# b-g-goodell/lattice-cryptography

Measured on NVIDIA B200. Metric: LM-OTS verifies/sec, higher is better.
Workload: dtype u32 (mod-q integer arithmetic, q < 2^16)

## Files before the change

lattice_cryptography_b200/csrc/api.cu:

```cuda
#include <cstdio>
#include <cstring>
#include <new>
#include <algorithm>
#include <cstdlib>
#include <string>
#include <vector>

#include <nvtx3/nvToolsExt.h>

#include "../../include/lcb200.h"
#include "engine.h"

using namespace lcb;

struct lcb_ctx {
    int device = 0;
    cudaStream_t stream = nullptr;
    bool own_stream = false;
    cudaStream_t copy_stream = nullptr;
    int secpar = 0, q = 0, d = 0, l = 0, rou = 0;
    RingCtx ring{};
    bool generic = false;
    bool wide = false;
    GenCtx gen{};
    uint32_t* d_gen_tab = nullptr;
    NttTables* d_tab = nullptr;
    uint32_t* d_a_hat = nullptr;
    bool has_key_ch = false;
    std::string last_error;
    int64_t launches = 0;
    uint8_t* idx_scratch = nullptr;
    size_t idx_scratch_bytes = 0;
    uint2* il_scratch = nullptr;
    size_t il_scratch_bytes = 0;
    uint32_t* d_mod_tab = nullptr;
    uint32_t* coop_scratch = nullptr;
    size_t coop_scratch_bytes = 0;
    bool profile = false;
    struct Pending { int id; cudaEvent_t a, b; };
    std::vector<Pending> pending;
    double prof_ms[24] = {0};
    int64_t prof_n[24] = {0};
};

namespace {

struct NvtxRange {
    explicit NvtxRange(const char* name) { nvtxRangePushA(name); }
    ~NvtxRange() { nvtxRangePop(); }
};
#define LCB_RANGE() NvtxRange nvtx_range_(__func__)

thread_local std::string g_create_error;

int fail(lcb_ctx* c, int status, const std::string& what) {
    if (c) c->last_error = what;
    return status;
}

int fail_cuda(lcb_ctx* c, cudaError_t e, const char* what) {
    return fail(c, e == cudaErrorMemoryAllocation ? LCB_ERR_OOM : LCB_ERR_CUDA,
                std::string(what) + ": " + cudaGetErrorString(e));
}

#define CK(c, call)                                              \
    do {                                                         \
        cudaError_t e_ = (call);                                 \
        if (e_ != cudaSuccess) return fail_cuda((c), e_, #call); \
    } while (0)

constexpr int64_t kPipeChunk = 1 << 17;

enum KernelId { K_SAMPLER = 0, K_SHAKE, K_NTT_FWD, K_NTT_INV, K_POLY_MUL, K_MATVEC, K_SIGN, K_VERIFY, K_ADDSUB,
                K_AGG_COEFS, K_AGG_PARTIAL, K_AGG_FINISH, K_AGGV_PARTIAL, K_AGGV_FINISH, K_PACK, K_UNPACK, K_GROUP_IDS,
                K_AGG_COEFS_SEG, K_AGG_PARTIAL_SEG, K_AGGV_PARTIAL_SEG, K_AGGV_RESIDUES, K_AGGV_LIMITS, K_AGG_FINISH_PACK,
                K_COUNT };
const char* const kKernelNames[K_COUNT] = {"sampler", "shake256", "ntt_fwd", "ntt_inv", "poly_mul", "matvec", "sign",
                                           "verify", "vec_addsub", "agg_coefs", "agg_partial", "agg_finish",
                                           "aggv_partial", "aggv_finish", "pack", "unpack", "group_ids",
                                           "agg_coefs_seg", "agg_partial_seg", "aggv_partial_seg", "aggv_residues",
                                           "aggv_limits", "agg_finish_pack"};
// ... 706 lines not shown
    m.q4 = 4 * uq;
    m.in_off = m.cq + 26 * uq + FP_BIAS;
    m.in_off_q4 = m.in_off + m.q4;
    m.bias_mod_q = FP_BIAS % uq;
    m.z1c = (int32_t)t.w[1] > (int32_t)m.half ? (int32_t)t.w[1] - (int32_t)uq : (int32_t)t.w[1];
    m.k1 = (uint32_t)((((1ull << 30) + (1ull << 15) + uq - 1) / uq) * uq);
    {
        uint64_t inv = uq;
        for (int it = 0; it < 6; ++it) inv *= 2 - (uint64_t)uq * inv;
        m.qinv_lo = (uint32_t)inv;
        m.qinv_hi = (uint32_t)(inv >> 32);
        const uint64_t lim = ~0ull / uq;
        m.dlim_lo = (uint32_t)lim;
        m.dlim_hi = (uint32_t)(lim >> 32);
        m.kq18 = (((1u << 18) + uq - 1) / uq) * uq;
        m.kw0 = (uint32_t)((uint64_t)(0x4B400000u + 2u) * uq);
    }
    for (int k = 0; k < 16; ++k) {
        c->ring.sc.w[k] = t.w[k];
        c->ring.sc.ws[k] = t.ws[k];
        c->ring.sc.iw[k] = t.iw[k];
        c->ring.sc.iws[k] = t.iws[k];
        c->ring.scf.w[k] = t.w[k];
        c->ring.scf.wq[k] = t.f_wq[k];
        c->ring.scf.cst[k] = t.f_cst[k];
        c->ring.scf.kw[k] = t.f_kw[k];
    }
    if ((e = cudaMalloc(&c->d_tab, sizeof(NttTables))) != cudaSuccess) return bail(e, "cudaMalloc tables");
    if ((e = cudaMemcpy(c->d_tab, &t, sizeof(NttTables), cudaMemcpyHostToDevice)) != cudaSuccess) return bail(e, "cudaMemcpy tables");
    if ((e = cudaMalloc(&c->d_a_hat, (size_t)l * D * sizeof(uint32_t))) != cudaSuccess) return bail(e, "cudaMalloc key_ch");
    c->ring.tab = c->d_tab;
    c->ring.a_hat = c->d_a_hat;
    c->gen.a_hat = c->d_a_hat;
    c->ring.l = l;
    c->ring.num_sms = prop.multiProcessorCount;
    {
        std::vector<uint32_t> mt(SAMPLER_MOD_TABLE_WORDS);
        fill_sampler_mod_table(mt.data());
        if ((e = cudaMalloc(&c->d_mod_tab, mt.size() * sizeof(uint32_t))) != cudaSuccess) return bail(e, "cudaMalloc sampler tables");
        if ((e = cudaMemcpy(c->d_mod_tab, mt.data(), mt.size() * sizeof(uint32_t), cudaMemcpyHostToDevice)) != cudaSuccess)
            return bail(e, "cudaMemcpy sampler tables");
    }
    *out = c;
    return LCB_OK;
}

int lcb_ctx_destroy(lcb_ctx* c) {
    if (!c) return LCB_OK;
    cudaSetDevice(c->device);
    if (c->stream) cudaStreamSynchronize(c->stream);
    if (c->d_tab) cudaFree(c->d_tab);
    if (c->d_gen_tab) cudaFree(c->d_gen_tab);
    if (c->d_a_hat) cudaFree(c->d_a_hat);
    if (c->idx_scratch) cudaFree(c->idx_scratch);
    if (c->d_mod_tab) cudaFree(c->d_mod_tab);
    if (c->il_scratch) cudaFree(c->il_scratch);
    if (c->coop_scratch) cudaFree(c->coop_scratch);
    if (c->own_stream && c->stream) cudaStreamDestroy(c->stream);
    if (c->copy_stream) {
        cudaStreamSynchronize(c->copy_stream);
        cudaStreamDestroy(c->copy_stream);
    }
    delete c;
    return LCB_OK;
}

int lcb_ctx_set_stream(lcb_ctx* c, void* cuda_stream) {
    if (!c) return LCB_ERR_INVALID;
    CK(c, cudaSetDevice(c->device));
    CK(c, cudaStreamSynchronize(c->stream));
    if (c->own_stream) cudaStreamDestroy(c->stream);
    c->stream = static_cast<cudaStream_t>(cuda_stream);
    c->own_stream = false;
    return LCB_OK;
}

int lcb_synchronize(lcb_ctx* c) {
    if (!c) return LCB_ERR_INVALID;
    CK(c, cudaSetDevice(c->device));
    CK(c, cudaStreamSynchronize(c->stream));
    return LCB_OK;
}

int lcb_ctx_root_of_unity(const lcb_ctx* c) { return c ? c->rou : LCB_ERR_INVALID; }

int64_t lcb_launch_count(const lcb_ctx* c) { return c ? c->launches : 0; }

static int profile_drain(lcb_ctx* c) {
    if (c->pending.empty()) return LCB_OK;
    CK(c, cudaStreamSynchronize(c->stream));
    for (auto& p : c->pending) {
        float ms = 0.f;
        if (cudaEventElapsedTime(&ms, p.a, p.b) == cudaSuccess) {
            c->prof_ms[p.id] += ms;
            c->prof_n[p.id] += 1;
        }
        cudaEventDestroy(p.a);
        cudaEventDestroy(p.b);
    }
    c->pending.clear();
    return LCB_OK;
}

int lcb_profile_enable(lcb_ctx* c, int on) {
    if (!c) return LCB_ERR_INVALID;
    CK(c, cudaSetDevice(c->device));
    int st = profile_drain(c);
    c->profile = on != 0;
    return st;
}

int lcb_profile_reset(lcb_ctx* c) {
    if (!c) return LCB_ERR_INVALID;
    CK(c, cudaSetDevice(c->device));
    int st = profile_drain(c);
    for (int i = 0; i < K_COUNT; ++i) { c->prof_ms[i] = 0; c->prof_n[i] = 0; }
    return st;
}

int lcb_profile_read(lcb_ctx* c, const char* kernel, double* total_ms, int64_t* launches) {
    if (!c || !kernel || !total_ms || !launches) return LCB_ERR_INVALID;
    CK(c, cudaSetDevice(c->device));
    int st = profile_drain(c);
    if (st != LCB_OK) return st;
    for (int i = 0; i < K_COUNT; ++i)
        if (std::strcmp(kernel, kKernelNames[i]) == 0) {
            *total_ms = c->prof_ms[i];
            *launches = c->prof_n[i];
            return LCB_OK;
        }
    return fail(c, LCB_ERR_INVALID, std::string("unknown kernel name ") + kernel);
}

int lcb_set_key_ch(lcb_ctx* c, const int16_t* key_ch_coef) {
    LCB_RANGE();
    if (!c || !key_ch_coef) return LCB_ERR_INVALID;
    CK(c, cudaSetDevice(c->device));
    Staging sg(c);
    const size_t cnt = (size_t)c->l * c->d;
    const int16_t* d_in;
    CK(c, sg.in(&d_in, key_ch_coef, cnt * ew(c)));
    uint16_t* d_ntt;
    CK(c, sg.alloc((void**)&d_ntt, cnt * ew(c) * sizeof(uint16_t)));
    if (c->generic) CK(c, timed(c, K_NTT_FWD, [&] { return g_launch_ntt_fwd(c->gen, d_in, c->l, d_ntt, c->stream); }));
    else CK(c, timed(c, K_NTT_FWD, [&] { return launch_ntt_fwd(c->ring, d_in, c->l, d_ntt, c->stream); }));
    if (c->wide) {
        CK(c, cudaMemcpyAsync(c->d_a_hat, d_ntt, cnt * sizeof(uint32_t), cudaMemcpyDeviceToDevice, c->stream));
        CK(c, cudaStreamSynchronize(c->stream));
    } else {
        std::vector<uint16_t> h16(cnt);
        CK(c, cudaMemcpyAsync(h16.data(), d_ntt, h16.size() * sizeof(uint16_t), cudaMemcpyDeviceToHost, c->stream));
        CK(c, cudaStreamSynchronize(c->stream));
        std::vector<uint32_t> h32(h16.begin(), h16.end());
        CK(c, cudaMemcpyAsync(c->d_a_hat, h32.data(), h32.size() * sizeof(uint32_t), cudaMemcpyHostToDevice, c->stream));
        CK(c, cudaStreamSynchronize(c->stream));
    }
    c->has_key_ch = true;
    CK(c, sg.finish());
    return LCB_OK;
}

int lcb_shake256_batch(lcb_ctx* c, const uint8_t* in, const int64_t* in_off, int64_t n, uint8_t* out,
                       int64_t out_len) {
    LCB_RANGE();
    if (!c || !in_off || !out || n < 0 || out_len < 0) return LCB_ERR_INVALID;
    if (n == 0 || out_len == 0) return LCB_OK;
    CK(c, cudaSetDevice(c->device));
    int64_t total = 0;
    CK(c, last_offset(c, in, in_off, n, &total));
    Staging sg(c);
    const uint8_t* d_in;
    const int64_t* d_off;
    uint8_t* d_out;
    CK(c, sg.in(&d_in, in, (size_t)total));
    CK(c, sg.in(&d_off, in_off, (size_t)n + 1));
    CK(c, sg.out(&d_out, out, (size_t)(n * out_len)));
    CK(c, timed(c, K_SHAKE, [&] { return launch_shake256(d_in, d_off, n, d_out, out_len, c->stream); }));
    CK(c, sg.finish());
    return LCB_OK;
}

int lcb_expand_seeds(lcb_ctx* c, const uint8_t* secret32, int64_t first, int64_t n, uint8_t* seeds) {
    LCB_RANGE();
    if (!c || !secret32 || !seeds || n < 0 || first < 0) return LCB_ERR_INVALID;
    if (c->secpar > 512 || (c->secpar & 7)) return fail(c, LCB_ERR_INVALID, "seed expansion needs secpar to be a multiple of 8, at most 512");
    if (n == 0) return LCB_OK;
    CK(c, cudaSetDevice(c->device));
    Staging sg(c);
    uint8_t* d_secret;
    uint8_t* d_out;
    CK(c, sg.alloc((void**)&d_secret, 32, true));
    CK(c, cudaMemcpyAsync(d_secret, secret32, 32, cudaMemcpyDefault, c->stream));
    CK(c, sg.out(&d_out, seeds, (size_t)n * c->secpar, true));
    CK(c, timed(c, K_SHAKE, [&] { return launch_seed_expand(d_secret, first, n, c->secpar, d_out, c->stream); }));
    CK(c, sg.finish());
    if (!on_device(secret32)) CK(c, cudaStreamSynchronize(c->stream));
    return LCB_OK;
}

int lcb_hash2polyvec_batch(lcb_ctx* c, const char* salt, const uint8_t* msgs, const int64_t* msg_off, int64_t n,
                           int bd, int wt, int vec_len, int16_t* out_dense, int16_t* out_pairs) {
    LCB_RANGE();
    if (!c || !msg_off || n < 0) return LCB_ERR_INVALID;
    if (n == 0) return LCB_OK;
    CK(c, cudaSetDevice(c->device));
    SamplerArgs a{};
    int st = fill_sampler(c, a, salt, nullptr, bd, wt, vec_len);
    if (st != LCB_OK) return fail(c, st, "bad sampler parameters");
    int64_t total = 0;
    CK(c, last_offset(c, msgs, msg_off, n, &total));
// ... 179 lines not shown
    CK(c, sg.out(&d_sig, sig, (size_t)n * l * D_));
    CK(c, sg.alloc((void**)&d_pairs, (size_t)n * sch->ch_wt * 2 * ew(c) * sizeof(int16_t)));
    int st = run_challenge(c, sch, d_msg, d_off, n, d_pairs);
    if (st != LCB_OK) return st;
    CK(c, timed(c, K_SIGN, [&] {
        return c->generic ? g_launch_sign(c->gen, d_sk, d_pairs, sch->ch_wt, n, d_sig, c->stream)
                          : launch_sign(c->ring, d_sk, d_pairs, sch->ch_wt, n, d_sig, c->stream);
    }));
    CK(c, sg.finish());
    return LCB_OK;
}

int lcb_lm_verify_batch(lcb_ctx* c, const lcb_scheme* sch, const uint16_t* vk_ntt, const uint8_t* chmsg,
                        const int64_t* chmsg_off, const int16_t* sig, const uint16_t* st_ntt, int64_t n, int bd,
                        int wt, uint8_t* verdict) {
    LCB_RANGE();
    if (!c || !sch || !vk_ntt || !chmsg_off || !sig || !verdict || n < 0 || bd < 0 || wt < 0) return LCB_ERR_INVALID;
    if (!c->has_key_ch) return fail(c, LCB_ERR_NO_KEY_CH, "lcb_lm_verify_batch before lcb_set_key_ch");
    if (n > ((int64_t)1 << 30)) return fail(c, LCB_ERR_INVALID, "more than 2^30 items in one verify call");
    if (n == 0) return LCB_OK;
    CK(c, cudaSetDevice(c->device));
    const int l = c->l;
    int64_t total = 0;
    CK(c, last_offset(c, chmsg, chmsg_off, n, &total));
    Staging sg(c);
    const uint16_t *d_vk, *d_st;
    const uint8_t* d_msg;
    const int64_t* d_off;
    const int16_t* d_sig;
    int16_t* d_pairs;
    uint8_t* d_verdict;
    const size_t D_ = (size_t)c->d * ew(c);
    CK(c, sg.in(&d_vk, vk_ntt, (size_t)n * 2 * D_));
    CK(c, sg.in(&d_msg, chmsg, (size_t)total));
    CK(c, sg.in(&d_off, chmsg_off, (size_t)n + 1));
    bool piped = false;
    CK(c, sg.in_piped(&d_sig, sig, (size_t)n * l * D_, &piped));
    CK(c, sg.in(&d_st, st_ntt, (size_t)n * D_));
    CK(c, sg.out(&d_verdict, verdict, (size_t)n));
    CK(c, sg.alloc((void**)&d_pairs, (size_t)n * sch->ch_wt * 2 * ew(c) * sizeof(int16_t)));
    const int vbd = bd > 32767 ? 32767 : bd;
    const int64_t chunk = piped && n > kPipeChunk ? kPipeChunk : n;
    std::vector<cudaEvent_t> arrived;
    if (piped) {
        CK(c, sg.pipe_begin());
        for (int64_t first = 0; first < n; first += chunk) {
            const int64_t m = n - first < chunk ? n - first : chunk;
            cudaEvent_t ev;
            CK(c, sg.pipe_chunk(d_sig + (size_t)first * l * D_, sig + (size_t)first * l * D_,
                                (size_t)m * l * D_ * sizeof(int16_t), &ev));
            arrived.push_back(ev);
        }
    }
    for (int64_t first = 0, k = 0; first < n; first += chunk, ++k) {
        const int64_t m = n - first < chunk ? n - first : chunk;
        int16_t* pairs = d_pairs + (size_t)first * sch->ch_wt * 2 * ew(c);
        int st = run_challenge(c, sch, d_msg, d_off + first, m, pairs);
        if (st != LCB_OK) return st;
        if (piped) CK(c, cudaStreamWaitEvent(c->stream, arrived[k], 0));
        CK(c, timed(c, K_VERIFY, [&] {
            if (c->generic)
                return g_launch_verify(c->gen, d_sig + (size_t)first * l * D_, d_vk + (size_t)first * 2 * D_, pairs, sch->ch_wt,
                                       nullptr, d_st ? d_st + (size_t)first * D_ : nullptr, m, bd, wt, d_verdict + first, c->stream);
            return launch_verify(c->ring, d_sig + (size_t)first * l * D_, d_vk + (size_t)first * 2 * D_, pairs, sch->ch_wt,
                                 nullptr, d_st ? d_st + (size_t)first * D_ : nullptr, m, vbd, wt, d_verdict + first,
                                 c->stream);
        }));
    }
    CK(c, sg.finish());
    return LCB_OK;
}

int lcb_pack_batch(lcb_ctx* c, const void* values, int64_t npoly, int bits, int bias, uint8_t* packed,
                   uint8_t* in_range) {
    LCB_RANGE();
    if (!c || !values || !packed || npoly < 0 || bits < 1 || bits > 16 || bias < 0 || bias > 65535) return LCB_ERR_INVALID;
    if (c->generic) return fail(c, LCB_ERR_INVALID, "the packed wire format is defined for d == 256, q < 2^16 contexts only");
    if (npoly == 0) return LCB_OK;
    CK(c, cudaSetDevice(c->device));
    Staging sg(c);
    const uint16_t* d_in;
    uint8_t *d_out, *d_ok;
    CK(c, sg.in(&d_in, static_cast<const uint16_t*>(values), (size_t)npoly * D));
    CK(c, sg.out(&d_out, packed, (size_t)npoly * 32 * bits));
    CK(c, sg.out(&d_ok, in_range, (size_t)npoly));
    if (reinterpret_cast<uintptr_t>(d_out) & 3u) return fail(c, LCB_ERR_INVALID, "packed buffer must be 4-byte aligned");
    CK(c, timed(c, K_PACK, [&] { return launch_pack(c->ring, d_in, npoly, bits, bias, d_out, d_ok, c->stream); }));
    CK(c, sg.finish());
    return LCB_OK;
}

int lcb_unpack_batch(lcb_ctx* c, const uint8_t* packed, int64_t npoly, int bits, int bias, void* values) {
    LCB_RANGE();
    if (!c || !values || !packed || npoly < 0 || bits < 1 || bits > 16 || bias < 0 || bias > 65535) return LCB_ERR_INVALID;
    if (c->generic) return fail(c, LCB_ERR_INVALID, "the packed wire format is defined for d == 256, q < 2^16 contexts only");
    if (npoly == 0) return LCB_OK;
    CK(c, cudaSetDevice(c->device));
    Staging sg(c);
    const uint8_t* d_in;
    uint16_t* d_out;
    CK(c, sg.in(&d_in, packed, (size_t)npoly * 32 * bits));
    CK(c, sg.out(&d_out, static_cast<uint16_t*>(values), (size_t)npoly * D));
    if (reinterpret_cast<uintptr_t>(d_in) & 3u) return fail(c, LCB_ERR_INVALID, "packed buffer must be 4-byte aligned");
    CK(c, timed(c, K_UNPACK, [&] { return launch_unpack(c->ring, d_in, npoly, bits, bias, d_out, c->stream); }));
    CK(c, sg.finish());
    return LCB_OK;
}

}

namespace {

int verify_packed(lcb_ctx* c, const lcb_scheme* sch, const uint8_t* vk_packed, int vk_bits, const uint8_t* chmsg,
// ... 903 lines not shown
```

lattice_cryptography_b200/csrc/engine.h:

```cpp
#pragma once
#include <cstdint>
#include <cuda_runtime.h>
#include "lcb_device.cuh"

namespace lcb {

constexpr int SALT_BYTES = 48;

struct SamplerArgs {
    const uint8_t* msgs;
    const int64_t* off;
    int64_t n;
    int64_t shared_len;
    int64_t index_first;
    int shared_msg;
    alignas(8) uint8_t salt[SALT_BYTES];
    int salt_len;
    alignas(8) uint8_t salt2[SALT_BYTES];
    int salt2_len;
    int paired;
    int secpar, bd, wt, vec_len;
    int idx_bits;
    int mag_bits;
    int pad_bits;
// ... 50 lines not shown
    const uint32_t* a_hat;
    int l, num_sms;
    bool wide;
};

cudaError_t g_launch_ntt_fwd(const GenCtx& c, const void* coef, int64_t npoly, void* out, cudaStream_t st);
cudaError_t g_launch_ntt_inv(const GenCtx& c, const void* in, int64_t npoly, void* coef, cudaStream_t st);
cudaError_t g_launch_poly_mul(const GenCtx& c, const void* a, const void* b, int64_t npoly, void* out, cudaStream_t st);
cudaError_t g_launch_ref_repr(const GenCtx& c, const void* coef, int64_t npoly, void* out, cudaStream_t st);
cudaError_t g_launch_matvec(const GenCtx& c, const void* vec_coef, int64_t nvec, void* vec_ntt, void* y_ntt, void* y_coef,
                            cudaStream_t st);
cudaError_t g_launch_sign(const GenCtx& c, const void* sk_ntt, const void* ch_pairs, int ch_wt, int64_t n, void* sig,
                          cudaStream_t st);
cudaError_t g_launch_verify(const GenCtx& c, const void* vec_coef, const void* vk_ntt, const void* ch_pairs, int ch_wt,
                            const void* rhs_only, const void* extra_rhs, int64_t n, int64_t bd, int wt, uint8_t* verdict,
                            cudaStream_t st);
cudaError_t g_launch_vec_addsub(const GenCtx& c, const void* a, const void* b, int64_t nelem, int sub, void* out,
                                cudaStream_t st);
cudaError_t g_launch_agg_partial(const GenCtx& c, const void* sigs, const void* ag_pairs, int64_t count, void* partial,
                                 cudaStream_t st);
cudaError_t g_launch_agg_partial_poly(const GenCtx& c, const void* sigs, const void* ag_pairs, int ag_wt, int64_t count,
                                      void* partial, cudaStream_t st);
cudaError_t g_launch_aggv_partial_poly(const GenCtx& c, const void* vk_ntt, const void* ch_pairs, int ch_wt, const void* ag_pairs,
                                       int ag_wt, int64_t count, void* partial, cudaStream_t st);
cudaError_t g_launch_agg_finish(const GenCtx& c, const void* partial, void* ag_sig, cudaStream_t st);
cudaError_t g_launch_aggv_partial(const GenCtx& c, const void* vk_ntt, const void* ch_pairs, int ch_wt, const void* ag_pairs,
                                  int64_t count, void* partial, cudaStream_t st);
cudaError_t g_launch_aggv_finish(const GenCtx& c, const void* partial, const void* ag_sig, int64_t total, int64_t ag_cap,
                                 int64_t avf_bd, int avf_wt, uint8_t* verdict, cudaStream_t st);

struct RingCtx {
    ModQ m;
    StageConst sc;
    StageConstF scf;
    StageConstF iscf;
    const NttTables* tab;
    const uint32_t* a_hat;
    int l;
    int num_sms;
};

cudaError_t launch_ntt_fwd(const RingCtx& c, const int16_t* coef, int64_t npoly, uint16_t* out, cudaStream_t st);
cudaError_t launch_ntt_ref_repr(const RingCtx& c, const int16_t* coef, int64_t npoly, int16_t* out, cudaStream_t st);
cudaError_t launch_ntt_inv(const RingCtx& c, const uint16_t* in, int64_t npoly, int16_t* coef, cudaStream_t st);
cudaError_t launch_poly_mul(const RingCtx& c, const int16_t* a, const int16_t* b, int64_t npoly, int16_t* out,
                            cudaStream_t st);
cudaError_t launch_matvec(const RingCtx& c, const int16_t* vec_coef, int64_t nvec, uint16_t* vec_ntt,
                          uint16_t* y_ntt, int16_t* y_coef, cudaStream_t st);
cudaError_t launch_sign(const RingCtx& c, const uint16_t* sk_ntt, const int16_t* ch_pairs, int ch_wt, int64_t n,
                        int16_t* sig, cudaStream_t st);
cudaError_t launch_verify(const RingCtx& c, const int16_t* vec_coef, const uint16_t* vk_ntt,
                          const int16_t* ch_pairs, int ch_wt, const uint16_t* rhs_only, const uint16_t* extra_rhs,
                          int64_t n, int bd, int wt, uint8_t* verdict, cudaStream_t st);
cudaError_t launch_verify_packed(const RingCtx& c, const uint8_t* sig_packed, int sig_bits, int sig_bias,
                                 const uint8_t* vk_packed, int vk_bits, const int16_t* ch_pairs, int ch_wt, int64_t n,
                                 int bd, int wt, uint8_t* verdict, cudaStream_t st, const uint8_t* st_packed = nullptr);
cudaError_t launch_sign_packed(const RingCtx& c, const uint16_t* sk_ntt, const int16_t* ch_pairs, int ch_wt, int64_t n,
                               int sig_bits, int sig_bias, uint8_t* sig_packed, uint8_t* in_range, cudaStream_t st);
cudaError_t launch_vec_addsub(const RingCtx& c, const int16_t* a, const int16_t* b, int64_t nelem, int sub,
                              int16_t* out, cudaStream_t st);
cudaError_t launch_agg_partial(const RingCtx& c, const int16_t* sigs, const int16_t* ag_pairs, int64_t count,
                               int32_t* partial, cudaStream_t st);
cudaError_t launch_agg_finish(const RingCtx& c, const int32_t* partial, int16_t* ag_sig, cudaStream_t st);
cudaError_t launch_aggv_partial(const RingCtx& c, const uint16_t* vk_ntt, const int16_t* ch_pairs, int ch_wt,
                                const int16_t* ag_pairs, int64_t count, int32_t* partial, cudaStream_t st);
cudaError_t launch_aggv_finish(const RingCtx& c, const int32_t* partial, const int16_t* ag_sig, int64_t total,
                               int ag_cap, int avf_bd, int avf_wt, uint8_t* verdict, cudaStream_t st);
cudaError_t launch_agg_partial_seg(const RingCtx& c, const void* sigs, int sig_bits, int sig_bias, const int16_t* ag_pairs,
                                   const int32_t* gid, int64_t total, int64_t n_agg, int32_t* partial, cudaStream_t st);
cudaError_t launch_agg_finish_n(const RingCtx& c, const int32_t* partial, int64_t nelem, int16_t* ag_sig, cudaStream_t st);
cudaError_t launch_aggv_partial_seg(const RingCtx& c, const void* vk_ntt, int vk_bits, const int16_t* ch_pairs, int ch_wt,
                                    const int16_t* ag_pairs, const int32_t* gid, int64_t total, int64_t n_agg,
                                    int32_t* partial, cudaStream_t st);
cudaError_t launch_aggv_residues(const RingCtx& c, const int32_t* partial, int64_t nelem, uint16_t* out, cudaStream_t st);
cudaError_t launch_aggv_limits(const RingCtx& c, const int64_t* agg_off, int64_t n_agg, const int16_t* ag_sig, int64_t ag_cap,
                               uint8_t* verdict, cudaStream_t st);
cudaError_t launch_aggv_limits_packed(const RingCtx& c, const int64_t* agg_off, int64_t n_agg, const uint8_t* ag_packed, int bits,
                                      int bias, int64_t ag_cap, uint8_t* verdict, cudaStream_t st);
cudaError_t launch_verify_rhs_packed(const RingCtx& c, const uint8_t* vec_packed, int bits, int bias, const uint16_t* rhs_only,
                                     int64_t n, int bd, int wt, uint8_t* verdict, cudaStream_t st);

cudaError_t launch_pack(const RingCtx& c, const void* in, int64_t npoly, int bits, int bias, uint8_t* out,
                        uint8_t* in_range, cudaStream_t st);
cudaError_t launch_unpack(const RingCtx& c, const uint8_t* in, int64_t npoly, int bits, int bias, void* out,
                          cudaStream_t st);
cudaError_t launch_agg_finish_pack(const RingCtx& c, const int32_t* partial, int64_t npoly, int bits, int bias, uint8_t* out,
                                   uint8_t* in_range, cudaStream_t st);

}
```

lattice_cryptography_b200/csrc/ring.cu:

```cuda
#include <cstdlib>

#include "engine.h"

namespace lcb {

namespace {

constexpr int RBS = 128;
constexpr int HWB = RBS / LANES;
#ifdef LCB_EXP_MBS
constexpr int MBS = LCB_EXP_MBS;
#else
constexpr int MBS = 512;
#endif
constexpr int MHWB = MBS / LANES;

struct HalfWarp {
    int lane;
    int slot;
    uint32_t* xb;
    unsigned mask;
};

__device__ __forceinline__ HalfWarp half_warp(uint32_t* xbase) {
// ... 1099 lines not shown
                const uint32_t hi = w + 1 < words ? __ldg(p + w + 1) : 0u;
                nz = (__funnelshift_r(__ldg(p + w), hi, (unsigned)pos & 31u) & mask) != bias;
            }
            ok = nz;
        }
        if (!ok) verdict[g] = 0;
    }
}

__global__ void __launch_bounds__(32) k_aggv_finish(ModQ m, StageConst sc, const NttTables* __restrict__ tab,
                                                    const uint32_t* __restrict__ a_hat, int l,
                                                    const int32_t* __restrict__ partial,
                                                    const int16_t* __restrict__ ag_sig, int64_t total, int ag_cap,
                                                    int avf_bd, int avf_wt, uint8_t* __restrict__ verdict) {
    __shared__ __align__(16) uint32_t xbuf[XWARP];
    const HalfWarp h = half_warp(xbuf);
    LaneTw tw;
    load_lane_tw(tw, tab->w, tab->ws, h.lane);
    uint64_t acc[EPT];
#pragma unroll
    for (int i = 0; i < EPT; ++i) acc[i] = 0;
    int maxabs = 0, maxw = 0;
    for (int i = 0; i < l; ++i) {
        const int16_t* p = ag_sig + i * D;
        uint32_t r[EPT];
        int nz = 0;
#pragma unroll
        for (int j = 0; j < EPT; ++j) {
            int x = __ldg(p + h.lane + 16 * j);
            maxabs = max(maxabs, abs(x));
            nz += (x != 0);
            r[j] = (uint32_t)(x + (int)m.cq);
        }
#pragma unroll
        for (int o = 8; o >= 1; o >>= 1) nz += __shfl_xor_sync(0xFFFFFFFFu, nz, o);
        maxw = max(maxw, nz);
        ntt_fwd_256(r, m, sc, tw, h.xb, h.lane);
#pragma unroll
        for (int g = 0; g < EPT; ++g) acc[g] += (uint64_t)r[g] * __ldg(a_hat + i * D + 16 * h.lane + g);
    }
#pragma unroll
    for (int o = 8; o >= 1; o >>= 1) maxabs = max(maxabs, __shfl_xor_sync(0xFFFFFFFFu, maxabs, o));
    bool ok = maxabs >= 1 && maxabs <= avf_bd && maxw >= 1 && maxw <= avf_wt && total >= 1 && total <= ag_cap;
#pragma unroll
    for (int k = 0; k < EPT; ++k) {
        int v = partial[16 * h.lane + k] % (int)m.q;
        if (v < 0) v += (int)m.q;
        ok &= reduce64(acc[k], m) == (uint32_t)v;
    }
    const unsigned votes = __ballot_sync(0xFFFFFFFFu, ok);
    if (threadIdx.x == 0) verdict[0] = (votes & 0xFFFFu) == 0xFFFFu ? 1 : 0;
}

template <typename K>
int resident_blocks(K kernel, int threads, size_t smem) {
    int nb = 0;
    if (cudaOccupancyMaxActiveBlocksPerMultiprocessor(&nb, kernel, threads, smem) != cudaSuccess || nb < 1) nb = 1;
    return nb;
}

inline unsigned persistent_grid(int64_t items, int per_block, int num_sms, int resident) {
    int64_t need = (items + per_block - 1) / per_block;
    int64_t cap = (int64_t)num_sms * resident;
    return (unsigned)(need < cap ? need : cap);
}

inline size_t ring_smem(int l, int threads = RBS) { return (size_t)l * AROW * 4 + (size_t)(threads / 32) * XWARP * 4; }
inline size_t matvec_smem(int l) { return ring_smem(l, MBS) + (size_t)MHWB * STAGE_HALF_BYTES + (size_t)TW_BYTES; }
inline size_t verify_smem(int l) {
    return ring_smem(l, VBS) + (size_t)VHWB * STAGE_HALF_BYTES + (size_t)TW_BYTES + (size_t)LANES * EPT * 4;
}

template <typename K>
cudaError_t allow_smem(K kernel, size_t smem) {
    return cudaFuncSetAttribute(kernel, cudaFuncAttributeMaxDynamicSharedMemorySize, (int)smem);
}

}

cudaError_t launch_ntt_fwd(const RingCtx& c, const int16_t* coef, int64_t npoly, uint16_t* out, cudaStream_t st) {
    if (npoly <= 0) return cudaSuccess;
    unsigned grid = persistent_grid(npoly, HWB, c.num_sms, resident_blocks(k_ntt_fwd, RBS, 0));
    k_ntt_fwd<<<grid, RBS, 0, st>>>(c.m, c.sc, c.tab, coef, npoly, out);
    return cudaGetLastError();
}

cudaError_t launch_ntt_ref_repr(const RingCtx& c, const int16_t* coef, int64_t npoly, int16_t* out, cudaStream_t st) {
    if (npoly <= 0) return cudaSuccess;
    unsigned grid = persistent_grid(npoly, HWB, c.num_sms, resident_blocks(k_ntt_ref_repr, RBS, 0));
    k_ntt_ref_repr<<<grid, RBS, 0, st>>>(c.m, c.sc, c.tab, coef, npoly, out);
    return cudaGetLastError();
}

cudaError_t launch_ntt_inv(const RingCtx& c, const uint16_t* in, int64_t npoly, int16_t* coef, cudaStream_t st) {
    if (npoly <= 0) return cudaSuccess;
    unsigned grid = persistent_grid(npoly, HWB, c.num_sms, resident_blocks(k_ntt_inv, RBS, 0));
    k_ntt_inv<<<grid, RBS, 0, st>>>(c.m, c.sc, c.tab, in, npoly, coef);
    return cudaGetLastError();
}

cudaError_t launch_poly_mul(const RingCtx& c, const int16_t* a, const int16_t* b, int64_t npoly, int16_t* out,
                            cudaStream_t st) {
    if (npoly <= 0) return cudaSuccess;
    unsigned grid = persistent_grid(npoly, HWB, c.num_sms, resident_blocks(k_poly_mul, RBS, 0));
    k_poly_mul<<<grid, RBS, 0, st>>>(c.m, c.sc, c.tab, a, b, npoly, out);
    return cudaGetLastError();
// ... 150 lines not shown
    const int64_t need = (total + AGG_WARPS * AGG_DEPTH - 1) / (AGG_WARPS * AGG_DEPTH);
    const int64_t ranges = seg_ranges(min(need, cap) * AGG_WARPS);
    const int64_t chunks = (ranges + AGG_WARPS - 1) / AGG_WARPS;
    const int64_t per_warp = (total + ranges - 1) / ranges;
    dim3 grid((unsigned)chunks, (unsigned)c.l);
    kern<<<grid, 32 * AGG_WARPS, 0, st>>>(c.m, c.l, static_cast<const int16_t*>(sigs), ag_pairs, gid, total, n_agg, per_warp,
                                          partial, sig_bias);
    return cudaGetLastError();
}

cudaError_t launch_aggv_partial_seg(const RingCtx& c, const void* vk_ntt, int vk_bits, const int16_t* ch_pairs, int ch_wt,
                                    const int16_t* ag_pairs, const int32_t* gid, int64_t total, int64_t n_agg,
                                    int32_t* partial, cudaStream_t st) {
    if (total <= 0) return cudaSuccess;
    if (vk_bits != 0 && vk_bits != 14) return cudaErrorNotSupported;
    auto kern = vk_bits == 14 ? k_aggv_partial_seg<14> : k_aggv_partial_seg<0>;
    int64_t blocks = (int64_t)persistent_grid(total, HWB, c.num_sms, resident_blocks(kern, RBS, 0));
    const int64_t ranges = seg_ranges(min(blocks, (int64_t)SEG_MAX_WARPS / HWB) * HWB);
    blocks = (ranges + HWB - 1) / HWB;
    const int64_t per_hw = (total + ranges - 1) / ranges;
    if (per_hw > ((int64_t)1 << 20)) return cudaErrorInvalidValue;
    kern<<<(unsigned)blocks, RBS, 0, st>>>(c.m, c.scf, c.tab, static_cast<const uint16_t*>(vk_ntt), ch_pairs, ch_wt, ag_pairs,
                                           gid, total, n_agg, per_hw, partial);
    return cudaGetLastError();
}

cudaError_t launch_aggv_residues(const RingCtx& c, const int32_t* partial, int64_t nelem, uint16_t* out, cudaStream_t st) {
    if (nelem <= 0) return cudaSuccess;
    const int64_t need = (nelem + 255) / 256;
    k_aggv_residues<<<(unsigned)min(need, (int64_t)c.num_sms * 16), 256, 0, st>>>(c.m, partial, nelem, out);
    return cudaGetLastError();
}

cudaError_t launch_aggv_limits(const RingCtx& c, const int64_t* agg_off, int64_t n_agg, const int16_t* ag_sig, int64_t ag_cap,
                               uint8_t* verdict, cudaStream_t st) {
    if (n_agg <= 0) return cudaSuccess;
    const int64_t need = (n_agg + 255) / 256;
    k_aggv_limits<<<(unsigned)min(need, (int64_t)c.num_sms * 16), 256, 0, st>>>(agg_off, n_agg, ag_sig, (int64_t)c.l * D / 8,
                                                                                ag_cap, verdict);
    return cudaGetLastError();
}

cudaError_t launch_aggv_limits_packed(const RingCtx& c, const int64_t* agg_off, int64_t n_agg, const uint8_t* ag_packed, int bits,
                                      int bias, int64_t ag_cap, uint8_t* verdict, cudaStream_t st) {
    if (n_agg <= 0) return cudaSuccess;
    if (bits < 1 || bits > 16) return cudaErrorInvalidValue;
    const int64_t need = (n_agg + 255) / 256;
    k_aggv_limits_packed<<<(unsigned)min(need, (int64_t)c.num_sms * 16), 256, 0, st>>>(
        agg_off, n_agg, reinterpret_cast<const uint32_t*>(ag_packed), (int64_t)c.l * D, bits, (uint32_t)bias & 0xFFFFu, ag_cap,
        verdict);
    return cudaGetLastError();
}

}
```

Before: 187.0 million.

## Add tcgen05 int8 tensor-core verify path with precomputed NTT-folded weight matrix

Adds a verify path for large batches when the challenge weight is at least the ring dimension. It folds the forward NTT of the signature and the multiply by the public a_hat into one precomputed int8 matrix, split into low and high bytes and cached per key. A persistent warp-specialised kernel streams signature tiles through TMA/cp.async pipelines into tcgen05 int8 MMAs that accumulate in TMEM, and fuses the bound check and the mod-q equality check in the epilogue. A separate kernel precomputes the right-hand side from the challenge and the verification key. This replaces per-item NTT arithmetic with dense matrix work, which costs much more raw arithmetic and a large weight image, plus risky hand-written PTX.

```diff
diff --git a/lattice_cryptography_b200/csrc/api.cu b/lattice_cryptography_b200/csrc/api.cu
--- a/lattice_cryptography_b200/csrc/api.cu
+++ b/lattice_cryptography_b200/csrc/api.cu
@@ -27,6 +27,9 @@
     NttTables* d_tab = nullptr;
     uint32_t* d_a_hat = nullptr;
     bool has_key_ch = false;
+    uint8_t* d_w_tc = nullptr;
+    uint64_t* d_cterm_tc = nullptr;
+    bool w_tc_ready = false;
     std::string last_error;
     int64_t launches = 0;
     uint8_t* idx_scratch = nullptr;
@@ -839,6 +842,8 @@
     if (c->d_tab) cudaFree(c->d_tab);
     if (c->d_gen_tab) cudaFree(c->d_gen_tab);
     if (c->d_a_hat) cudaFree(c->d_a_hat);
+    if (c->d_w_tc) cudaFree(c->d_w_tc);
+    if (c->d_cterm_tc) cudaFree(c->d_cterm_tc);
     if (c->idx_scratch) cudaFree(c->idx_scratch);
     if (c->d_mod_tab) cudaFree(c->d_mod_tab);
     if (c->il_scratch) cudaFree(c->il_scratch);
@@ -943,6 +948,7 @@
         CK(c, cudaStreamSynchronize(c->stream));
     }
     c->has_key_ch = true;
+    c->w_tc_ready = false;
     CK(c, sg.finish());
     return LCB_OK;
 }
@@ -1228,13 +1234,30 @@
             arrived.push_back(ev);
         }
     }
+    uint16_t* d_t = nullptr;
     for (int64_t first = 0, k = 0; first < n; first += chunk, ++k) {
         const int64_t m = n - first < chunk ? n - first : chunk;
         int16_t* pairs = d_pairs + (size_t)first * sch->ch_wt * 2 * ew(c);
         int st = run_challenge(c, sch, d_msg, d_off + first, m, pairs);
         if (st != LCB_OK) return st;
         if (piped) CK(c, cudaStreamWaitEvent(c->stream, arrived[k], 0));
+        const bool tc = !c->generic && wt >= c->d && m >= kVerifyTcMinBatch && l <= 64;
+        if (tc && !d_t) {
+            if (!c->d_w_tc) {
+                CK(c, cudaMalloc(&c->d_w_tc, verify_tc_w_bytes(l)));
+                CK(c, cudaMalloc(&c->d_cterm_tc, D_ * sizeof(uint64_t)));
+            }
+            if (!c->w_tc_ready) {
+                CK(c, launch_verify_tc_build(c->ring, (uint32_t)c->rou, c->d_w_tc, c->d_cterm_tc, c->stream));
+                c->w_tc_ready = true;
+            }
+            CK(c, sg.alloc((void**)&d_t, (size_t)chunk * D_ * sizeof(uint16_t)));
+        }
         CK(c, timed(c, K_VERIFY, [&] {
+            if (tc)
+                return launch_verify_tc(c->ring, c->d_w_tc, c->d_cterm_tc, d_sig + (size_t)first * l * D_,
+                                        d_vk + (size_t)first * 2 * D_, pairs, sch->ch_wt,
+                                        d_st ? d_st + (size_t)first * D_ : nullptr, m, vbd, d_t, d_verdict + first, c->stream);
             if (c->generic)
                 return g_launch_verify(c->gen, d_sig + (size_t)first * l * D_, d_vk + (size_t)first * 2 * D_, pairs, sch->ch_wt,
                                        nullptr, d_st ? d_st + (size_t)first * D_ : nullptr, m, bd, wt, d_verdict + first, c->stream);
diff --git a/lattice_cryptography_b200/csrc/engine.h b/lattice_cryptography_b200/csrc/engine.h
--- a/lattice_cryptography_b200/csrc/engine.h
+++ b/lattice_cryptography_b200/csrc/engine.h
@@ -126,6 +126,12 @@
 cudaError_t launch_verify(const RingCtx& c, const int16_t* vec_coef, const uint16_t* vk_ntt,
                           const int16_t* ch_pairs, int ch_wt, const uint16_t* rhs_only, const uint16_t* extra_rhs,
                           int64_t n, int bd, int wt, uint8_t* verdict, cudaStream_t st);
+constexpr int64_t kVerifyTcMinBatch = (int64_t)1 << 15;
+size_t verify_tc_w_bytes(int l);
+cudaError_t launch_verify_tc_build(const RingCtx& c, uint32_t psi, uint8_t* w_img, uint64_t* cterm, cudaStream_t st);
+cudaError_t launch_verify_tc(const RingCtx& c, const uint8_t* w_img, const uint64_t* cterm, const int16_t* sig,
+                             const uint16_t* vk_ntt, const int16_t* ch_pairs, int ch_wt, const uint16_t* extra_rhs,
+                             int64_t n, int bd, uint16_t* t_scratch, uint8_t* verdict, cudaStream_t st);
 cudaError_t launch_verify_packed(const RingCtx& c, const uint8_t* sig_packed, int sig_bits, int sig_bias,
                                  const uint8_t* vk_packed, int vk_bits, const int16_t* ch_pairs, int ch_wt, int64_t n,
                                  int bd, int wt, uint8_t* verdict, cudaStream_t st, const uint8_t* st_packed = nullptr);
diff --git a/lattice_cryptography_b200/csrc/ring.cu b/lattice_cryptography_b200/csrc/ring.cu
--- a/lattice_cryptography_b200/csrc/ring.cu
+++ b/lattice_cryptography_b200/csrc/ring.cu
@@ -1175,6 +1175,328 @@
     if (threadIdx.x == 0) verdict[0] = (votes & 0xFFFFu) == 0xFFFFu ? 1 : 0;
 }
 
+constexpr int TC_TM = 128;
+constexpr int TC_WN = 512;
+constexpr int TC_KC = 64;
+constexpr int TC_STAGES = 4;
+constexpr int TC_RAW = 6;
+constexpr int TC_A_STAGE = TC_TM * TC_KC;
+constexpr int TC_B_STAGE = TC_WN * TC_KC;
+constexpr int TC_THREADS = 320;
+constexpr int TC_MAX_L = 64;
+constexpr size_t TC_SMEM = (size_t)TC_STAGES * (TC_A_STAGE + TC_B_STAGE) + (size_t)TC_RAW * TC_A_STAGE +
+                           D * sizeof(uint64_t) + 2 * TC_TM + 1024;
+static_assert(255ll * 255 * 512 * TC_MAX_L < (1ll << 31), "acc_lo must fit int32");
+
+__host__ __device__ __forceinline__ uint32_t tc_img_off(int rows, int r, int k) {
+    return (uint32_t)((k >> 5) * rows * 32 + (r >> 3) * 256 + ((k >> 4) & 1) * 128 + (r & 7) * 16 + (k & 15));
+}
+
+__device__ __forceinline__ uint32_t tc_pow(uint32_t b, uint32_t e, uint32_t q) {
+    uint64_t r = 1, x = b;
+    for (; e; e >>= 1, x = x * x % q)
+        if (e & 1) r = r * x % q;
+    return (uint32_t)r;
+}
+
+__global__ void k_tc_build_w(uint32_t q, uint32_t psi, int l, const uint32_t* __restrict__ a_hat, uint8_t* __restrict__ w) {
+    const int64_t idx = (int64_t)blockIdx.x * blockDim.x + threadIdx.x;
+    if (idx >= (int64_t)D * D * l) return;
+    const int p = (int)(idx % D), k = (int)(idx / D), i = k >> 8, c = k & 255;
+    const uint32_t br = __brev((uint32_t)p) >> 24;
+    const uint32_t wv = (uint32_t)((uint64_t)a_hat[i * D + p] % q * tc_pow(psi, ((2 * br + 1) * c) & 511, q) % q);
+    const uint32_t v2[2] = {wv, (uint32_t)((uint64_t)wv * 256 % q)};
+#pragma unroll
+    for (int h = 0; h < 2; ++h) {
+        const int rep = v2[h] < 32768u ? (int)v2[h] : (int)v2[h] - (int)q;
+        const int kk = 2 * k + h;
+        uint8_t* blk = w + (size_t)(kk / TC_KC) * TC_B_STAGE;
+        blk[tc_img_off(TC_WN, p, kk % TC_KC)] = (uint8_t)(rep & 0xFF);
+        blk[tc_img_off(TC_WN, D + p, kk % TC_KC)] = (uint8_t)((rep >> 8) & 0xFF);
+    }
+}
+
+__global__ void k_tc_build_corr(uint32_t q, uint32_t psi, int l, const uint32_t* __restrict__ a_hat, uint64_t q40,
+                                uint64_t* __restrict__ cterm) {
+    const int p = blockIdx.x * blockDim.x + threadIdx.x;
+    if (p >= D) return;
+    const uint32_t br = __brev((uint32_t)p) >> 24;
+    const uint32_t wp = tc_pow(psi, 2 * br + 1, q);
+    uint64_t sum = 0;
+    for (int i = 0; i < l; ++i) {
+        uint64_t x = 1;
+        for (int c = 0; c < D; ++c, x = x * wp % q) sum += (uint64_t)a_hat[i * D + p] % q * x % q;
+    }
+    cterm[p] = q40 - sum % q * 32768 % q;
+}
+
+__global__ void __launch_bounds__(RBS) k_tc_rhs(ModQ m, StageConstF scf, const NttTables* __restrict__ tab,
+                                                const uint16_t* __restrict__ vk_ntt, const int16_t* __restrict__ ch_pairs,
+                                                int ch_wt, const uint16_t* __restrict__ extra_rhs, int64_t n,
+                                                uint16_t* __restrict__ t_out) {
+    extern __shared__ __align__(16) uint32_t smem[];
+    uint32_t* xbuf = smem;
+    uint4* twtab = reinterpret_cast<uint4*>(xbuf + (RBS / 32) * XWARP);
+    fill_tw_shared(twtab, tab);
+    const HalfWarp h = half_warp(xbuf);
+    const LaneTwFShared twf{twtab + h.lane * TW_ROW};
+    const int64_t first = (int64_t)blockIdx.x * HWB, stride = (int64_t)gridDim.x * HWB;
+    const int64_t trips = first < n ? (n - first + stride - 1) / stride : 0;
+    for (int64_t it = 0; it < trips; ++it) {
+        const int64_t raw = first + it * stride + h.slot;
+        const bool live = raw < n;
+        const int64_t item = live ? raw : n - 1;
+        int cx[EPT];
+        uint32_t c[EPT], vl[EPT], rhs[EPT];
+        load_pairs_raw(cx, ch_pairs + item * ch_wt * 2, ch_wt, h.xb, h.lane);
+        ntt_fwd_256_fp(cx, c, m, scf, twf, h.xb, h.lane);
+        load_u16x16(vl, vk_ntt + item * 2 * D + 16 * h.lane);
+        load_u16x16(rhs, vk_ntt + item * 2 * D + D + 16 * h.lane);
+        if (extra_rhs) {
+            uint32_t ex[EPT];
+            load_u16x16(ex, extra_rhs + item * D + 16 * h.lane);
+#pragma unroll
+            for (int k = 0; k < EPT; ++k) rhs[k] += ex[k];
+        }
+        uint32_t o[EPT / 2];
+#pragma unroll
+        for (int k = 0; k < EPT; k += 2) {
+            uint32_t t2[2];
+#pragma unroll
+            for (int u = 0; u < 2; ++u) {
+                const uint32_t cr = barrett_full(c[k + u] - FP_BIAS, m), w = barrett_full(m.cq2 - vl[k + u], m);
+                t2[u] = barrett_full(rhs[k + u] + m.q - barrett_full(cr * w, m), m);
+            }
+            o[k / 2] = t2[0] | (t2[1] << 16);
+        }
+        if (live) {
+            uint4* dst = reinterpret_cast<uint4*>(t_out + item * D + 16 * h.lane);
+            dst[0] = make_uint4(o[0], o[1], o[2], o[3]);
+            dst[1] = make_uint4(o[4], o[5], o[6], o[7]);
+        }
+    }
+}
+
+__device__ __forceinline__ uint32_t tc_smem(const void* p) { return (uint32_t)__cvta_generic_to_shared(p); }
+__device__ __forceinline__ void tc_wait(uint32_t bar, uint32_t parity) {
+#ifdef LCB_CHECKED
+    uint64_t t0 = 0;
+#endif
+    for (int spin = 0;; ++spin) {
+        uint32_t ok;
+        asm volatile("{ .reg .pred p; mbarrier.try_wait.parity.shared::cta.b64 p, [%1], %2; selp.u32 %0, 1, 0, p; }"
+                     : "=r"(ok) : "r"(bar), "r"(parity) : "memory");
+        if (ok) return;
+#ifdef LCB_CHECKED
+        uint64_t t;
+        asm volatile("mov.u64 %0, %%globaltimer;" : "=l"(t));
+        if (spin == 0) t0 = t;
+        LCB_CHECK(t - t0 < 4000000000ull);
+#endif
+    }
+}
+__device__ __forceinline__ void tc_arrive(uint32_t bar) { asm volatile("mbarrier.arrive.shared::cta.b64 _, [%0];" ::"r"(bar) : "memory"); }
+__device__ __forceinline__ uint64_t tc_desc(uint32_t addr) {
+    return (uint64_t)((addr >> 4) & 0x3FFF) | ((uint64_t)(128 >> 4) << 16) | ((uint64_t)(256 >> 4) << 32) | (1ull << 46);
+}
+__host__ __device__ constexpr uint32_t tc_idesc(bool b_signed) { return (2u << 4) | ((b_signed ? 1u : 0u) << 10) | ((256u >> 3) << 17) | ((128u >> 4) << 24); }
+
+__global__ void __launch_bounds__(TC_THREADS, 1) k_verify_tc(ModQ m, const uint8_t* __restrict__ w_img,
+                                                             const uint64_t* __restrict__ cterm, const int16_t* __restrict__ sig,
+                                                             const uint16_t* __restrict__ t_rhs, int l, int64_t n, int bd,
+                                                             uint8_t* __restrict__ verdict) {
+    extern __shared__ __align__(1024) uint8_t smem_raw[];
+    uint8_t* sm = reinterpret_cast<uint8_t*>((reinterpret_cast<uintptr_t>(smem_raw) + 1023) & ~(uintptr_t)1023);
+    uint8_t* sA = sm;
+    uint8_t* sB = sA + TC_STAGES * TC_A_STAGE;
+    uint8_t* sRaw = sB + TC_STAGES * TC_B_STAGE;
+    uint64_t* sC = reinterpret_cast<uint64_t*>(sRaw + TC_RAW * TC_A_STAGE);
+    uint8_t* sBad = reinterpret_cast<uint8_t*>(sC + D);
+    __shared__ __align__(8) uint64_t full[TC_STAGES], ready[TC_STAGES], empty[TC_STAGES], bnd[2], tfull, tempty;
+    __shared__ uint32_t tmem_base;
+    const int warp = threadIdx.x >> 5, lane = threadIdx.x & 31;
+    const int chunks = 8 * l;
+    const int tiles = (int)((n + TC_TM - 1) / TC_TM);
+    const int my_tiles = tiles > (int)blockIdx.x ? (tiles - 1 - (int)blockIdx.x) / (int)gridDim.x + 1 : 0;
+    if (threadIdx.x == 0) {
+        for (int s = 0; s < TC_STAGES; ++s) {
+            asm volatile("mbarrier.init.shared::cta.b64 [%0], 1;" ::"r"(tc_smem(&full[s])));
+            asm volatile("mbarrier.init.shared::cta.b64 [%0], 4;" ::"r"(tc_smem(&ready[s])));
+            asm volatile("mbarrier.init.shared::cta.b64 [%0], 1;" ::"r"(tc_smem(&empty[s])));
+        }
+        for (int b = 0; b < 2; ++b) asm volatile("mbarrier.init.shared::cta.b64 [%0], 4;" ::"r"(tc_smem(&bnd[b])));
+        asm volatile("mbarrier.init.shared::cta.b64 [%0], 1;" ::"r"(tc_smem(&tfull)));
+        asm volatile("mbarrier.init.shared::cta.b64 [%0], 4;" ::"r"(tc_smem(&tempty)));
+        asm volatile("fence.mbarrier_init.release.cluster;" ::: "memory");
+    }
+    for (int p = threadIdx.x; p < D; p += blockDim.x) sC[p] = cterm[p];
+    if (warp == 1) {
+        asm volatile("tcgen05.alloc.cta_group::1.sync.aligned.shared::cta.b32 [%0], 512;" ::"r"(tc_smem(&tmem_base)));
+        asm volatile("tcgen05.relinquish_alloc_permit.cta_group::1.sync.aligned;");
+    }
+    asm volatile("tcgen05.fence::before_thread_sync;" ::: "memory");
+    __syncthreads();
+    asm volatile("tcgen05.fence::after_thread_sync;" ::: "memory");
+    const uint32_t tmem = tmem_base;
+
+    if (warp == 0) {
+        if (lane == 0) {
+            int s = 0;
+            uint32_t ph = 0;
+            for (int t = 0; t < my_tiles; ++t)
+                for (int c = 0; c < chunks; ++c) {
+                    tc_wait(tc_smem(&empty[s]), ph ^ 1);
+                    const uint32_t fb = tc_smem(&full[s]);
+                    asm volatile("mbarrier.arrive.expect_tx.shared::cta.b64 _, [%0], %1;" ::"r"(fb), "r"(TC_B_STAGE) : "memory");
+                    asm volatile("cp.async.bulk.shared::cluster.global.mbarrier::complete_tx::bytes [%0], [%1], %2, [%3];"
+                                 ::"r"(tc_smem(sB + s * TC_B_STAGE)), "l"(w_img + (size_t)c * TC_B_STAGE), "r"(TC_B_STAGE), "r"(fb)
+                                 : "memory");
+                    if (++s == TC_STAGES) { s = 0; ph ^= 1; }
+                }
+        }
+    } else if (warp == 1) {
+        if (lane == 0) {
+            int s = 0;
+            uint32_t ph = 0;
+            for (int t = 0; t < my_tiles; ++t) {
+                tc_wait(tc_smem(&tempty), (t & 1) ^ 1);
+                asm volatile("tcgen05.fence::after_thread_sync;" ::: "memory");
+                for (int c = 0; c < chunks; ++c) {
+                    tc_wait(tc_smem(&full[s]), ph);
+                    tc_wait(tc_smem(&ready[s]), ph);
+                    asm volatile("tcgen05.fence::after_thread_sync;" ::: "memory");
+                    const uint32_t a0 = tc_smem(sA + s * TC_A_STAGE), b0 = tc_smem(sB + s * TC_B_STAGE);
+#pragma unroll
+                    for (int ks = 0; ks < TC_KC / 32; ++ks) {
+                        const uint64_t ad = tc_desc(a0 + ks * TC_TM * 32);
+                        const uint32_t acc = (c | ks) ? 1u : 0u;
+                        asm volatile("{ .reg .pred p; setp.ne.b32 p, %4, 0; tcgen05.mma.cta_group::1.kind::i8 [%0], %1, %2, %3, p; }"
+                                     ::"r"(tmem), "l"(ad), "l"(tc_desc(b0 + ks * TC_WN * 32)), "r"(tc_idesc(false)), "r"(acc));
+                        asm volatile("{ .reg .pred p; setp.ne.b32 p, %4, 0; tcgen05.mma.cta_group::1.kind::i8 [%0], %1, %2, %3, p; }"
+                                     ::"r"(tmem + 256), "l"(ad), "l"(tc_desc(b0 + ks * TC_WN * 32 + 256 * 32)), "r"(tc_idesc(true)),
+                                       "r"(acc));
+                    }
+                    asm volatile("tcgen05.commit.cta_group::1.mbarrier::arrive::one.shared::cluster.b64 [%0];"
+                                 ::"r"(tc_smem(&empty[s])) : "memory");
+                    if (++s == TC_STAGES) { s = 0; ph ^= 1; }
+                }
+                asm volatile("tcgen05.commit.cta_group::1.mbarrier::arrive::one.shared::cluster.b64 [%0];"
+                             ::"r"(tc_smem(&tfull)) : "memory");
+            }
+        }
+    } else if (warp >= 6) {
+        const int t = threadIdx.x - 6 * 32, pc = t & 3, r0 = t >> 2;
+        const int64_t row_bytes = (int64_t)l * D * 2;
+        const uint8_t* sig_b = reinterpret_cast<const uint8_t*>(sig);
+        const int total = my_tiles * chunks;
+        const uint32_t raw0 = tc_smem(sRaw) + 16u * (uint32_t)t;
+        auto issue = [&](int g) {
+            if (g < total) {
+                const int tile = (int)blockIdx.x + (g / chunks) * (int)gridDim.x, c = g % chunks;
+                const uint32_t dst = raw0 + (uint32_t)(g % TC_RAW) * TC_A_STAGE;
+#pragma unroll
+                for (int j = 0; j < 4; ++j) {
+                    int64_t item = (int64_t)tile * TC_TM + r0 + 32 * j;
+                    item = item < n ? item : n - 1;
+                    const uint8_t* src = sig_b + item * row_bytes + c * TC_KC + 16 * pc;
+                    LCB_CHECK(item >= 0 && c * TC_KC + 16 * pc + 16 <= row_bytes);
+                    asm volatile("cp.async.cg.shared.global [%0], [%1], 16;" ::"r"(dst + 2048u * j), "l"(src) : "memory");
+                }
+            }
+            asm volatile("cp.async.commit_group;" ::: "memory");
+        };
+        for (int g = 0; g < TC_RAW - 1; ++g) issue(g);
+        int s = 0;
+        uint32_t ph = 0;
+        uint32_t mx[4], mn[4];
+#pragma unroll
+        for (int j = 0; j < 4; ++j) { mx[j] = 0x80008000u; mn[j] = 0x7FFF7FFFu; }
+        for (int g = 0; g < total; ++g) {
+            issue(g + TC_RAW - 1);
+            asm volatile("cp.async.wait_group %0;" ::"n"(TC_RAW - 1) : "memory");
+            tc_wait(tc_smem(&empty[s]), ph ^ 1);
+            const uint4* raw = reinterpret_cast<const uint4*>(sRaw + (g % TC_RAW) * TC_A_STAGE + 16 * t);
+            uint8_t* dstA = sA + s * TC_A_STAGE;
+#pragma unroll
+            for (int j = 0; j < 4; ++j) {
+                uint4 v = raw[128 * j];
+                mx[j] = __vimax3_s16x2(mx[j], v.x, v.y); mx[j] = __vimax3_s16x2(mx[j], v.z, v.w);
+                mn[j] = __vimin3_s16x2(mn[j], v.x, v.y); mn[j] = __vimin3_s16x2(mn[j], v.z, v.w);
+                v.x ^= 0x80008000u; v.y ^= 0x80008000u; v.z ^= 0x80008000u; v.w ^= 0x80008000u;
+                *reinterpret_cast<uint4*>(dstA + tc_img_off(TC_TM, r0 + 32 * j, 16 * pc)) = v;
+            }
+            asm volatile("fence.proxy.async.shared::cta;" ::: "memory");
+            __syncwarp();
+            if (lane == 0) tc_arrive(tc_smem(&ready[s]));
+            if (++s == TC_STAGES) { s = 0; ph ^= 1; }
+            if (g % chunks == chunks - 1) {
+                const int tt = g / chunks;
+#pragma unroll
+                for (int j = 0; j < 4; ++j) {
+                    uint32_t a = mx[j], b = mn[j];
+                    a = __vmaxs2(a, __shfl_xor_sync(0xFFFFFFFFu, a, 1)); a = __vmaxs2(a, __shfl_xor_sync(0xFFFFFFFFu, a, 2));
+                    b = __vmins2(b, __shfl_xor_sync(0xFFFFFFFFu, b, 1)); b = __vmins2(b, __shfl_xor_sync(0xFFFFFFFFu, b, 2));
+                    const int hi = max((int)(int16_t)(a & 0xFFFF), (int)(int16_t)(a >> 16));
+                    const int lo = min((int)(int16_t)(b & 0xFFFF), (int)(int16_t)(b >> 16));
+                    if (pc == 0) sBad[(tt & 1) * TC_TM + r0 + 32 * j] = (hi > bd || lo < -bd) ? 1 : 0;
+                    mx[j] = 0x80008000u;
+                    mn[j] = 0x7FFF7FFFu;
+                }
+                __syncwarp();
+                if (lane == 0) tc_arrive(tc_smem(&bnd[tt & 1]));
+            }
+        }
+        asm volatile("cp.async.wait_group 0;" ::: "memory");
+    } else {
+        const int row = 32 * (warp & 3) + lane;
+        const uint32_t lane_addr = tmem + ((uint32_t)(32 * (warp & 3)) << 16);
+        for (int t = 0; t < my_tiles; ++t) {
+            const int64_t item = ((int64_t)blockIdx.x + (int64_t)t * gridDim.x) * TC_TM + row;
+            const int64_t it_c = item < n ? item : n - 1;
+            tc_wait(tc_smem(&tfull), t & 1);
+            tc_wait(tc_smem(&bnd[t & 1]), (t >> 1) & 1);
+            asm volatile("tcgen05.fence::after_thread_sync;" ::: "memory");
+            bool ok = sBad[(t & 1) * TC_TM + row] == 0;
+            const uint4* trow = reinterpret_cast<const uint4*>(t_rhs + it_c * D);
+            for (int p0 = 0; p0 < D; p0 += 32) {
+                uint32_t lo[32], hi[32];
+#define TC_LD32(dst, addr)                                                                                              \
+    asm volatile("tcgen05.ld.sync.aligned.32x32b.x32.b32 {%0,%1,%2,%3,%4,%5,%6,%7,%8,%9,%10,%11,%12,%13,%14,%15,"       \
+                 "%16,%17,%18,%19,%20,%21,%22,%23,%24,%25,%26,%27,%28,%29,%30,%31}, [%32];"                              \
+                 : "=r"(dst[0]), "=r"(dst[1]), "=r"(dst[2]), "=r"(dst[3]), "=r"(dst[4]), "=r"(dst[5]), "=r"(dst[6]),     \
+                   "=r"(dst[7]), "=r"(dst[8]), "=r"(dst[9]), "=r"(dst[10]), "=r"(dst[11]), "=r"(dst[12]), "=r"(dst[13]), \
+                   "=r"(dst[14]), "=r"(dst[15]), "=r"(dst[16]), "=r"(dst[17]), "=r"(dst[18]), "=r"(dst[19]),            \
+                   "=r"(dst[20]), "=r"(dst[21]), "=r"(dst[22]), "=r"(dst[23]), "=r"(dst[24]), "=r"(dst[25]),            \
+                   "=r"(dst[26]), "=r"(dst[27]), "=r"(dst[28]), "=r"(dst[29]), "=r"(dst[30]), "=r"(dst[31])             \
+                 : "r"(addr))
+                TC_LD32(lo, lane_addr + (uint32_t)p0);
+                TC_LD32(hi, lane_addr + 256u + (uint32_t)p0);
+#undef TC_LD32
+                asm volatile("tcgen05.wait::ld.sync.aligned;" ::: "memory");
+#pragma unroll
+                for (int v = 0; v < 4; ++v) {
+                    const uint4 tv = __ldg(trow + p0 / 8 + v);
+                    const uint32_t tw[4] = {tv.x, tv.y, tv.z, tv.w};
+#pragma unroll
+                    for (int u = 0; u < 8; ++u) {
+                        const int j = 8 * v + u;
+                        const int64_t prod = (int64_t)(int32_t)lo[j] + 256 * (int64_t)(int32_t)hi[j];
+                        const uint64_t x = (uint64_t)prod + sC[p0 + j] - ((tw[u >> 1] >> (16 * (u & 1))) & 0xFFFFu);
+                        ok &= divisible_by_q(x, m);
+                    }
+                }
+            }
+            asm volatile("tcgen05.fence::before_thread_sync;" ::: "memory");
+            __syncwarp();
+            if (lane == 0) tc_arrive(tc_smem(&tempty));
+            if (item < n) verdict[item] = ok ? 1 : 0;
+        }
+    }
+    asm volatile("tcgen05.fence::before_thread_sync;" ::: "memory");
+    __syncthreads();
+    if (warp == 1) asm volatile("tcgen05.dealloc.cta_group::1.sync.aligned.b32 %0, 512;" ::"r"(tmem));
+}
+
 template <typename K>
 int resident_blocks(K kernel, int threads, size_t smem) {
     int nb = 0;
@@ -1431,4 +1753,33 @@
     return cudaGetLastError();
 }
 
-}
+size_t verify_tc_w_bytes(int l) { return (size_t)8 * l * TC_B_STAGE; }
+
+cudaError_t launch_verify_tc_build(const RingCtx& c, uint32_t psi, uint8_t* w_img, uint64_t* cterm, cudaStream_t st) {
+    if (c.l > TC_MAX_L) return cudaErrorInvalidValue;
+    const int64_t total = (int64_t)D * D * c.l;
+    k_tc_build_w<<<(unsigned)((total + 255) / 256), 256, 0, st>>>(c.m.q, psi, c.l, c.a_hat, w_img);
+    const uint64_t q = c.m.q, q40 = (((uint64_t)1 << 40) + q - 1) / q * q;
+    k_tc_build_corr<<<1, D, 0, st>>>(c.m.q, psi, c.l, c.a_hat, q40, cterm);
+    return cudaGetLastError();
+}
+
+cudaError_t launch_verify_tc(const RingCtx& c, const uint8_t* w_img, const uint64_t* cterm, const int16_t* sig,
+                             const uint16_t* vk_ntt, const int16_t* ch_pairs, int ch_wt, const uint16_t* extra_rhs,
+                             int64_t n, int bd, uint16_t* t_scratch, uint8_t* verdict, cudaStream_t st) {
+    if (n <= 0) return cudaSuccess;
+    if (c.l > TC_MAX_L || n > ((int64_t)1 << 30)) return cudaErrorInvalidValue;
+    const size_t rsmem = (size_t)(RBS / 32) * XWARP * 4 + (size_t)TW_BYTES;
+    cudaError_t e = allow_smem(k_tc_rhs, rsmem);
+    if (e != cudaSuccess) return e;
+    unsigned grid = persistent_grid(n, HWB, c.num_sms, resident_blocks(k_tc_rhs, RBS, rsmem));
+    k_tc_rhs<<<grid, RBS, rsmem, st>>>(c.m, c.scf, c.tab, vk_ntt, ch_pairs, ch_wt, extra_rhs, n, t_scratch);
+    if ((e = cudaGetLastError()) != cudaSuccess) return e;
+    if ((e = allow_smem(k_verify_tc, TC_SMEM)) != cudaSuccess) return e;
+    const int64_t tiles = (n + TC_TM - 1) / TC_TM;
+    grid = (unsigned)(tiles < c.num_sms ? tiles : c.num_sms);
+    k_verify_tc<<<grid, TC_THREADS, TC_SMEM, st>>>(c.m, w_img, cterm, sig, t_scratch, c.l, n, bd, verdict);
+    return cudaGetLastError();
+}
+
+}
```

Result: slower. 167.1 million (median of 6 runs) (-10.7%).
